# liyi14/mx-DeepIM

Hardware: NVIDIA H100
Metric: 480x640 4-iter pose refinements/sec (higher is better)
Workload: dtype fp16

## Files before the change

### mx-deepim_b200/csrc/conv_igemm.cuh

```cuda
#pragma once
#include <cuda.h>
#include <cuda_fp16.h>
#include "common.cuh"
#include "wgmma.cuh"

namespace dim {

struct ConvKParams {
  CUtensorMap a_map[4];
  CUtensorMap a_lo_map[4];
  CUtensorMap b_map;
  CUtensorMap b_lo_map;
  int KH, KW, stride, cchunks;
  int BW, BH, n_col_tiles;
  int Hq, Ho, Wo, Bn;
  int out_Hp, out_Wp, out_py, out_px, Cout;
  int kblocks;
  float slope;
  const float *bias;
  __nv_bfloat16 *out_hi, *out_lo;
  int in_off_r, in_off_c;
  int out_sy, out_sx, out_oy, out_ox, out_H, out_W, out_cs, out_coff;
  struct PixBuf { const __nv_bfloat16 *p; int Hp, Wp, py, px, cs, coff; } addend, mask;
  int mask_climit;
};

namespace ptx {
// ... 57 lines not shown
        : "memory");
}
__device__ __forceinline__ void tma_load_3d(void *dst, const CUtensorMap *map, uint64_t *bar, int c0, int c1, int c2) {
  if (elect_one())
    asm volatile(
        "cp.async.bulk.tensor.3d.shared::cluster.global.mbarrier::complete_tx::bytes [%0], [%1, {%3, %4, %5}], [%2];" ::
            "r"(smem_u32(dst)),
        "l"((uint64_t)map), "r"(smem_u32(bar)), "r"(c0), "r"(c1), "r"(c2)
        : "memory");
}

__device__ __forceinline__ void mbar_arrive(uint64_t *bar) {
  asm volatile("mbarrier.arrive.shared::cta.b64 _, [%0];" ::"r"(smem_u32(bar)) : "memory");
}

__device__ __forceinline__ void tma_load_4d(void *dst, const CUtensorMap *map, uint64_t *bar, int c0, int c1, int c2, int c3) {
  if (elect_one())
    asm volatile(
        "cp.async.bulk.tensor.4d.shared::cluster.global.mbarrier::complete_tx::bytes [%0], [%1, {%3, %4, %5, %6}], [%2];" ::
            "r"(smem_u32(dst)),
        "l"((uint64_t)map), "r"(smem_u32(bar)), "r"(c0), "r"(c1), "r"(c2), "r"(c3)
        : "memory");
}

__device__ __forceinline__ uint64_t gmma_desc(uint32_t saddr, uint32_t lbo_bytes, uint32_t sbo_bytes, uint32_t layout) {
  uint64_t d = 0;
  d |= (uint64_t)((saddr & 0x3FFFFu) >> 4);
  d |= (uint64_t)((lbo_bytes >> 4) & 0x3FFFu) << 16;
  d |= (uint64_t)((sbo_bytes >> 4) & 0x3FFFu) << 32;
  d |= (uint64_t)layout << 62;
// ... 11 lines not shown
  asm("cvt.rn.satfinite.f16x2.f32 %0, %1, %2;" : "=r"(r) : "f"(b), "f"(a));
  return r;
}
__device__ __forceinline__ uint32_t pack2_bf16(float a, float b) {
  uint32_t r;
  asm("cvt.rn.bf16x2.f32 %0, %1, %2;" : "=r"(r) : "f"(b), "f"(a));
  return r;
}

constexpr int kConv1Slack = 2048;


__device__ __forceinline__ int frag_row(int t) { return ((t >> 5) << 4) + ((t & 31) >> 2); }

template <bool SPLIT3, bool F16>
__device__ __forceinline__ void store_pair(float v0, float v1, float2 b, float slope, __nv_bfloat16 *out_hi, __nv_bfloat16 *out_lo,
                                           long long off) {
  v0 += b.x;
  v1 += b.y;
  v0 = v0 > 0.f ? v0 : v0 * slope;
  v1 = v1 > 0.f ? v1 : v1 * slope;
  if (F16) {
    *reinterpret_cast<uint32_t *>(out_hi + off) = pack2_f16(v0, v1);
  } else {
    const uint32_t h = pack2_bf16(v0, v1);
    *reinterpret_cast<uint32_t *>(out_hi + off) = h;
    if (SPLIT3)
      *reinterpret_cast<uint32_t *>(out_lo + off) = pack2_bf16(v0 - __uint_as_float(h << 16), v1 - __uint_as_float(h & 0xFFFF0000u));
  }
}

__device__ __forceinline__ void store_pair_generic(float v0, float v1, const ConvKParams &p, int n, bool valid, long long off,
                                                   long long add_off, long long mask_off) {
  if (!valid || n >= p.Cout) return;
  if (p.bias) {
    v0 += __ldg(p.bias + n);
    v1 += __ldg(p.bias + n + 1);
  }
  if (p.addend.p) {
    const __nv_bfloat162 a = *reinterpret_cast<const __nv_bfloat162 *>(p.addend.p + add_off);
    v0 += __low2float(a);
    v1 += __high2float(a);
  }
  if (p.mask.p) {
// ... 146 lines not shown
          const bool valid = (m < p.BW * p.BH) && (n_img < p.Bn) && (oh < p.Ho) && (ow < p.Wo);
          if (valid) {
            const long long off = (((long long)n_img * p.out_Hp + oh + p.out_py) * p.out_Wp + ow + p.out_px) * p.Cout + n0 + q2;
#pragma unroll
            for (int j = 0; j < BLOCK_N / 8; ++j)
              store_pair<SPLIT3, F16>(acc[4 * j + 2 * rr], acc[4 * j + 2 * rr + 1],
                                      make_float2(__ldg(p.bias + n0 + 8 * j + q2), __ldg(p.bias + n0 + 8 * j + q2 + 1)), p.slope, p.out_hi,
                                      p.out_lo, off + 8 * j);
          }
        }
      }
    }
  }
}

template <int STAGES, bool SPLIT3, bool F16>
__global__ void __launch_bounds__(384, 1) conv1_kernel(const __grid_constant__ ConvKParams p, const int rows_total,
                                                       const int rows_per_chunk, const int chunks_per_col,
                                                       const int strip_bytes ) {
  constexpr int NPREC = SPLIT3 ? 2 : 1;
  constexpr int B_BYTES = 64 * 32 * 2, RES_BYTES = 16 * B_BYTES * NPREC;
  extern __shared__ uint8_t smem_raw[];
  uint8_t *smem = reinterpret_cast<uint8_t *>((reinterpret_cast<uintptr_t>(smem_raw) + 1023) & ~(uintptr_t)1023);
  uint8_t *res = smem;
  uint8_t *ring = smem + RES_BYTES;
  const int stage_bytes = strip_bytes * NPREC;
  uint64_t *full_bar = reinterpret_cast<uint64_t *>(ring + STAGES * stage_bytes + kConv1Slack);
  uint64_t *empty_bar = full_bar + STAGES;
  uint64_t *res_bar = empty_bar + STAGES;

  const int wgi = threadIdx.x >> 7, warp = threadIdx.x >> 5;
  const int R = p.BW + 3;
  const uint32_t LBO = (uint32_t)R * 16u;
  const int ct = blockIdx.x / chunks_per_col, ck = blockIdx.x - ct * chunks_per_col;
  const int g_lo = ck * rows_per_chunk;
  const int g_hi = min(rows_total, g_lo + rows_per_chunk);
  const int n_rows = max(0, g_hi - g_lo);
  const int n_strips = n_rows > 0 ? n_rows + 3 : 0;
  const int ow0 = ct * p.BW;

  if (threadIdx.x == 0) {
    for (int s = 0; s < STAGES; ++s) {
      ptx::mbar_init(&full_bar[s], 1);
      ptx::mbar_init(&empty_bar[s], 2);
    }
    ptx::mbar_init(res_bar, 1);
    ptx::fence_barrier_init();
    ptx::prefetch_tmap(&p.b_map);
    ptx::prefetch_tmap(&p.a_map[0]);
  }
  __syncthreads();

  if (wgi == 0) {
    ptx::regs_producer();
    if (warp == 0 && n_rows > 0) {
      if (ptx::elect_one()) {
        ptx::mbar_expect_tx_raw(res_bar, (uint32_t)RES_BYTES);
        for (int kb = 0; kb < 16; ++kb) {
          ptx::tma_load_2d_raw(res + kb * B_BYTES, &p.b_map, res_bar, kb * 32, 0);
          if (SPLIT3) ptx::tma_load_2d_raw(res + (16 + kb) * B_BYTES, &p.b_lo_map, res_bar, kb * 32, 0);
        }
      }
      __syncwarp();
      const uint32_t tx = (uint32_t)(R * 64) * NPREC;
      for (int s = 0; s < n_strips; ++s) {
        const int slot = s % STAGES;
        ptx::mbar_wait(&empty_bar[slot], (((uint32_t)(s / STAGES)) & 1u) ^ 1u);
        uint8_t *st = ring + slot * stage_bytes;
        ptx::mbar_expect_tx(&full_bar[slot], tx);
        ptx::tma_load_4d(st, &p.a_map[0], &full_bar[slot], 0, ow0, 0, g_lo + s);
        if (SPLIT3) ptx::tma_load_4d(st + strip_bytes, &p.a_lo_map[0], &full_bar[slot], 0, ow0, 0, g_lo + s);
      }
    }
  } else if (n_rows > 0) {
    ptx::regs_consumer();
    const int set = wgi - 1, t = threadIdx.x & 127;
    const bool arriver = t == 0;
    const int r0 = frag_row(t), q2 = (t & 3) * 2;
    float2 bias[8];
#pragma unroll
    for (int j = 0; j < 8; ++j) bias[j] = make_float2(__ldg(p.bias + 8 * j + q2), __ldg(p.bias + 8 * j + q2 + 1));
    const uint32_t ring_a = ptx::smem_u32(ring);
    const uint64_t dring = ptx::gmma_desc(ring_a, LBO, 128, ptx::kNoSwizzle);
    const uint64_t dring3 = ptx::gmma_desc(ring_a, 2u * LBO, 128, ptx::kNoSwizzle) + 3u;
    const uint64_t lo_step = (uint64_t)((uint32_t)strip_bytes >> 4);
    const uint64_t slot_step = (uint64_t)((uint32_t)stage_bytes >> 4);
    const uint64_t kstep = (uint64_t)(2u * LBO >> 4);
    const uint64_t dres = ptx::gmma_desc(ptx::smem_u32(res), 16, 512, ptx::kSW64);
    const uint64_t dres_lo = dres + (uint64_t)((16 * B_BYTES) >> 4);
    const int n_cols_valid = min(p.BW, p.Wo - ow0);
    ptx::mbar_wait(res_bar, 0);
    if (set == 1 && arriver) ptx::mbar_arrive(&empty_bar[0]);
    for (int row = set; row < n_rows; row += 2) {
      float acc[2][32];
#pragma unroll
      for (int dh = 0; dh < 4; ++dh) {
        const int s = row + dh;
        ptx::mbar_wait(&full_bar[s % STAGES], ((uint32_t)(s / STAGES)) & 1u);
      }
      wg::fence_acc(acc[0]);
      wg::fence_acc(acc[1]);
      wg::fence();
#pragma unroll
      for (int h = 0; h < 2; ++h) {
#pragma unroll
        for (int dh = 0; dh < 4; ++dh) {
          const uint64_t so = (uint64_t)((row + dh) % STAGES) * slot_step + (uint64_t)(h * 64);
#pragma unroll
          for (int k = 0; k < 2; ++k) {
#pragma unroll
            for (int dw = 0; dw < 4; ++dw) {
              if ((dh == 3 || dw == 3) && k == 1) continue;
              const uint64_t da = (dw == 3 ? dring3 : dring + (uint64_t)dw + (uint64_t)k * kstep) + so;
              const uint64_t wo = (uint64_t)((dh * 4 + dw) * (B_BYTES >> 4) + 2 * k);
              wg::mma<64, F16, 0, 0>(acc[h], da, dres + wo, (dh | dw | k) ? 1u : 0u);
              if (SPLIT3) {
                wg::mma<64, false, 0, 0>(acc[h], da + lo_step, dres + wo, 1u);
                wg::mma<64, false, 0, 0>(acc[h], da, dres_lo + wo, 1u);
              }
            }
          }
        }
      }
      wg::commit();
      wg::wait<0>();
      wg::fence_acc(acc[0]);
      wg::fence_acc(acc[1]);
      if (arriver) {
        ptx::mbar_arrive(&empty_bar[row % STAGES]);
        ptx::mbar_arrive(&empty_bar[(row + 1) % STAGES]);
      }
      const int g = g_lo + row;
      const int n_img = g / p.Hq, oh = g - n_img * p.Hq;
      if (n_img < p.Bn && oh < p.Ho) {
        const long long row_off = (((long long)n_img * p.out_Hp + oh + p.out_py) * p.out_Wp + ow0 + p.out_px) * 64 + q2;
#pragma unroll
        for (int h = 0; h < 2; ++h)
#pragma unroll
          for (int rr = 0; rr < 2; ++rr) {
            const int m = h * 64 + r0 + rr * 8;
            if (m < n_cols_valid) {
#pragma unroll
              for (int j = 0; j < 8; ++j)
                store_pair<SPLIT3, F16>(acc[h][4 * j + 2 * rr], acc[h][4 * j + 2 * rr + 1], bias[j], p.slope, p.out_hi, p.out_lo,
                                        row_off + (long long)m * 64 + 8 * j);
            }
          }
      }
    }
  }
}

template <int STAGES, bool SPLIT3, bool F16, int NB>
__global__ void __launch_bounds__(384, 1) conv1_rgbd_kernel(const __grid_constant__ ConvKParams p, const int rows_total,
                                                            const int rows_per_chunk, const int chunks_per_col,
                                                            const int strip_bytes ) {
  constexpr int NPREC = SPLIT3 ? 2 : 1;
  constexpr int TAP_BYTES = NB * 128, RES_BYTES = 16 * TAP_BYTES * NPREC;
  extern __shared__ uint8_t smem_raw[];
  uint8_t *smem = reinterpret_cast<uint8_t *>((reinterpret_cast<uintptr_t>(smem_raw) + 1023) & ~(uintptr_t)1023);
  uint8_t *res = smem;
  uint8_t *ring = smem + RES_BYTES;
  const int stage_bytes = strip_bytes * NPREC;
  uint64_t *full_bar = reinterpret_cast<uint64_t *>(ring + STAGES * stage_bytes + kConv1Slack);
// ... 131 lines not shown
```

### mx-deepim_b200/csrc/net.cu

```cuda
#include <cuda_fp16.h>
#include <string.h>

#include <mutex>

#include "launch.cuh"
#include "net_state.cuh"

namespace dim {

static void build_geometry(NetState *ns, int H, int W) {
  int h = H, w = W;
  for (int i = 0; i < 10; ++i) {
    const LayerSpec &s = kLayers[i];
    LayerGeom &g = ns->g[i];
    g.Cin = s.Cin; g.Cout = s.Cout; g.k = s.k; g.stride = s.stride; g.pad = s.pad;
    g.Hin = h; g.Win = w;
    g.Ho = (h + 2 * s.pad - s.k) / s.stride + 1;
    g.Wo = (w + 2 * s.pad - s.k) / s.stride + 1;
    if (g.Ho < 1) g.Ho = 1;
    if (g.Wo < 1) g.Wo = 1;
    int Hp = h + 2 * s.pad, Wp = w + 2 * s.pad;
    if (s.stride == 2) { Hp += Hp & 1; Wp += Wp & 1; }
    g.py = g.px = s.pad;
    if (i == 0 && ns->input_depth) {
// ... 71 lines not shown
  for (int i = 0; i < 10; ++i) {
    const LayerGeom &g = ns->g[i];
    ConvKParams &kp = tm.kp[i];
    memset(&kp, 0, sizeof(kp));
    for (int lo = 0; lo < 2; ++lo) {
      __nv_bfloat16 *base = lo ? ns->act_lo[i] : ns->act_hi[i];
      CUtensorMap *maps = lo ? kp.a_lo_map : kp.a_map;
      const uint32_t box[3] = {(uint32_t)g.BLOCK_K, (uint32_t)g.BW, (uint32_t)g.BH};
      if (i == 0 && ns->input_depth) {
        const uint64_t dims[4] = {8, (uint64_t)g.cols, 8, (uint64_t)B * g.rows};
        const uint64_t str[3] = {16, (uint64_t)g.cols * 16, (uint64_t)g.cols * 128};
        const uint32_t box4[4] = {8, (uint32_t)(g.BW + 3), 8, 1};
        if (int rc = encode_map(&maps[0], base, 4, dims, str, box4, 0)) return rc;
        maps[1] = maps[2] = maps[3] = maps[0];
      } else if (i == 0) {
        const uint64_t dims[4] = {8, (uint64_t)g.cols, 4, (uint64_t)B * g.rows};
        const uint64_t str[3] = {16, (uint64_t)g.cols * 16, (uint64_t)g.cols * 64};
        const uint32_t box4[4] = {8, (uint32_t)(g.BW + 3), 4, 1};
        if (int rc = encode_map(&maps[0], base, 4, dims, str, box4, 0)) return rc;
        maps[1] = maps[2] = maps[3] = maps[0];
      } else if (g.stride_eff == 1) {
        const uint64_t dims[3] = {(uint64_t)g.Cbuf, (uint64_t)g.cols, (uint64_t)B * g.rows};
        const uint64_t str[2] = {(uint64_t)g.Cbuf * 2, (uint64_t)g.cols * g.Cbuf * 2};
        if (int rc = encode_map(&maps[0], base, 3, dims, str, box, g.BLOCK_K)) return rc;
        maps[1] = maps[2] = maps[3] = maps[0];
      } else {
        for (int ph = 0; ph < 2; ++ph)
          for (int pw = 0; pw < 2; ++pw) {
            const uint64_t dims[3] = {(uint64_t)g.Cbuf, (uint64_t)g.cols / 2, (uint64_t)B * g.rows / 2};
            const uint64_t str[2] = {(uint64_t)2 * g.Cbuf * 2, (uint64_t)2 * g.cols * g.Cbuf * 2};
            __nv_bfloat16 *vb = base + ((size_t)ph * g.cols + pw) * g.Cbuf;
            if (int rc = encode_map(&maps[(ph << 1) | pw], vb, 3, dims, str, box, g.BLOCK_K)) return rc;
          }
      }
    }
// ... 9 lines not shown
    kp.KH = g.KH; kp.KW = g.KW; kp.stride = g.stride_eff; kp.cchunks = g.Ceff / g.BLOCK_K;
    kp.BW = g.BW; kp.BH = g.BH; kp.n_col_tiles = g.n_col_tiles;
    kp.Hq = g.Hq; kp.Ho = g.Ho; kp.Wo = g.Wo; kp.Bn = B;
    if (i < 9) {
      const LayerGeom &nx = ns->g[i + 1];
      kp.out_Hp = nx.rows; kp.out_Wp = nx.cols; kp.out_py = nx.py; kp.out_px = nx.px;
    } else {
      kp.out_Hp = g.Ho; kp.out_Wp = g.Wo; kp.out_py = 0; kp.out_px = 0;
    }
    kp.Cout = g.Cout;
    kp.kblocks = g.kblocks;
    kp.slope = 0.1f;
    kp.bias = ns->bias[i];
    kp.out_hi = ns->act_hi[i + 1];
    kp.out_lo = ns->act_lo[i + 1];
  }
  return 0;
}

template <bool F16>
__device__ __forceinline__ void mma_bf16_16816(float *c, const uint32_t *a, uint32_t b0, uint32_t b1) {
  if (F16)
    asm volatile(
        "mma.sync.aligned.m16n8k16.row.col.f32.f16.f16.f32 {%0,%1,%2,%3}, {%4,%5,%6,%7}, {%8,%9}, {%0,%1,%2,%3};"
        : "+f"(c[0]), "+f"(c[1]), "+f"(c[2]), "+f"(c[3])
        : "r"(a[0]), "r"(a[1]), "r"(a[2]), "r"(a[3]), "r"(b0), "r"(b1));
  else
    asm volatile(
        "mma.sync.aligned.m16n8k16.row.col.f32.bf16.bf16.f32 {%0,%1,%2,%3}, {%4,%5,%6,%7}, {%8,%9}, {%0,%1,%2,%3};"
        : "+f"(c[0]), "+f"(c[1]), "+f"(c[2]), "+f"(c[3])
// ... 281 lines not shown
template <int BN, int ST, bool S3, bool F16>
static int launch_conv(const ConvKParams &kp, int total_tiles, int n_tiles, int cap, cudaStream_t st) {
  using S = ConvSmem2<BN, ST, S3>;
  static bool attr_set = false;
  if (!attr_set) {
    DIM_CHECK(cudaFuncSetAttribute(conv_igemm_persistent_kernel<BN, ST, S3, F16>, cudaFuncAttributeMaxDynamicSharedMemorySize,
                                   S::TOTAL));
    attr_set = true;
  }
  const int grid = total_tiles < cap ? total_tiles : cap;
  conv_igemm_persistent_kernel<BN, ST, S3, F16><<<grid, 384, S::TOTAL, st>>>(kp, total_tiles, n_tiles);
  DIM_LAUNCH_CHECK();
  return 0;
}

template <int ST, bool S3, bool F16>
static int launch_conv1(const ConvKParams &kp, int grid, int rows_total, int rpc, int chunks, int strip_bytes, cudaStream_t st) {
  const int smem_bytes = (S3 ? 2 : 1) * 16 * 4096 + ST * (S3 ? 2 : 1) * strip_bytes + kConv1Slack + 1024 + 256;
  DIM_REQUIRE(smem_bytes <= 227 * 1024, "conv1: image too wide for the rolling-strip ring");
  static int set = 0;
  if (set < smem_bytes) {
    DIM_CHECK(cudaFuncSetAttribute(conv1_kernel<ST, S3, F16>, cudaFuncAttributeMaxDynamicSharedMemorySize, smem_bytes));
    set = smem_bytes;
  }
  conv1_kernel<ST, S3, F16><<<grid, 384, smem_bytes, st>>>(kp, rows_total, rpc, chunks, strip_bytes);
  DIM_LAUNCH_CHECK();
  return 0;
}

template <int ST, bool S3, bool F16, int NB>
static int launch_conv1_rgbd(const ConvKParams &kp, int grid, int rows_total, int rpc, int chunks, int strip_bytes,
                             cudaStream_t st) {
  const int smem_bytes = 16 * NB * 128 * (S3 ? 2 : 1) + ST * (S3 ? 2 : 1) * strip_bytes + kConv1Slack + 1024 + 256;
  DIM_REQUIRE(smem_bytes <= 227 * 1024, "conv1 (RGB-D): image too wide for the rolling-strip ring");
  static int set = 0;
  if (set < smem_bytes) {
    DIM_CHECK(cudaFuncSetAttribute(conv1_rgbd_kernel<ST, S3, F16, NB>, cudaFuncAttributeMaxDynamicSharedMemorySize,
                                   smem_bytes));
    set = smem_bytes;
  }
// ... 62 lines not shown
    int rc;
    if (i == 0 && ns->input_depth) {
      const int nsplit = s3 ? 4 : 1;
      const int rows_total = B * g.Hq;
      int chunks = sms / (g.n_col_tiles * nsplit);
      if (chunks > cdiv(rows_total, 16)) chunks = cdiv(rows_total, 16);
      if (chunks < 1) chunks = 1;
      const int rpc = cdiv(rows_total, chunks);
      chunks = cdiv(rows_total, rpc);
      const int strip_bytes = cdiv((g.BW + 3) * 128, 128) * 128;
      const int grid = g.n_col_tiles * chunks * nsplit;
      rc = s3 ? launch_conv1_rgbd<5, true, false, 16>(kp, grid, rows_total, rpc, chunks, strip_bytes, st)
              : (f16 ? launch_conv1_rgbd<6, false, true, 64>(kp, grid, rows_total, rpc, chunks, strip_bytes, st)
                     : launch_conv1_rgbd<6, false, false, 64>(kp, grid, rows_total, rpc, chunks, strip_bytes, st));
    } else if (i == 0) {
      const int rows_total = B * g.Hq;
      int chunks = sms / g.n_col_tiles;
      if (chunks > cdiv(rows_total, 16)) chunks = cdiv(rows_total, 16);
      if (chunks < 1) chunks = 1;
      const int rpc = cdiv(rows_total, chunks);
      chunks = cdiv(rows_total, rpc);
      const int strip_bytes = cdiv((g.BW + 3) * 64, 128) * 128;
      const int grid = g.n_col_tiles * chunks;
      rc = s3 ? launch_conv1<5, true, false>(kp, grid, rows_total, rpc, chunks, strip_bytes, st)
              : (f16 ? launch_conv1<8, false, true>(kp, grid, rows_total, rpc, chunks, strip_bytes, st)
                     : launch_conv1<8, false, false>(kp, grid, rows_total, rpc, chunks, strip_bytes, st));
    } else if (g.BLOCK_N == 128) {
      rc = s3 ? launch_conv<128, 3, true, false>(kp, total_tiles, n_tiles, sms, st)
              : (f16 ? launch_conv<128, 6, false, true>(kp, total_tiles, n_tiles, sms, st)
                     : launch_conv<128, 6, false, false>(kp, total_tiles, n_tiles, sms, st));
    } else {
      rc = s3 ? launch_conv<256, 2, true, false>(kp, total_tiles, n_tiles, sms, st)
              : (f16 ? launch_conv<256, 4, false, true>(kp, total_tiles, n_tiles, sms, st)
                     : launch_conv<256, 4, false, false>(kp, total_tiles, n_tiles, sms, st));
    }
    if (rc) return rc;
    if (ns->layer_events && i < 9) DIM_CHECK(cudaEventRecord(ns->layer_events[i + 1], st));
  }
  if (ns->layer_events) DIM_CHECK(cudaEventRecord(ns->layer_events[10], st));
  if (after_conv) DIM_CHECK(cudaEventRecord(after_conv, st));
  if (s3)
// ... 63 lines not shown
```

### mx-deepim_b200/csrc/wgmma.cuh

```cuda
#pragma once
#include <stdint.h>

namespace dim {
namespace wg {

__device__ __forceinline__ void fence() { asm volatile("wgmma.fence.sync.aligned;" ::: "memory"); }
__device__ __forceinline__ void commit() { asm volatile("wgmma.commit_group.sync.aligned;" ::: "memory"); }
template <int N>
__device__ __forceinline__ void wait() { asm volatile("wgmma.wait_group.sync.aligned %0;" ::"n"(N) : "memory"); }

template <int R>
__device__ __forceinline__ void fence_acc(float (&d)[R]) {
#pragma unroll
  for (int i = 0; i < R; ++i) asm volatile("" : "+f"(d[i])::"memory");
}

template <int N, bool F16, int TA, int TB>
__device__ __forceinline__ void mma(float (&d)[N / 2], uint64_t da, uint64_t db, uint32_t scale_d);

template <>
__device__ __forceinline__ void mma<16, false, 0, 0>(float (&d)[8], uint64_t da, uint64_t db, uint32_t scale_d) {
  asm volatile(
      "{\n.reg .pred p;\nsetp.ne.b32 p, %10, 0;\n"
      "wgmma.mma_async.sync.aligned.m64n16k16.f32.bf16.bf16 {%0, %1, %2, %3, %4, %5, %6, %7}, %8, %9, p, 1, 1, 0, 0;\n}\n"
// ... 44 lines not shown
      "wgmma.mma_async.sync.aligned.m64n64k16.f32.f16.f16 {%0, %1, %2, %3, %4, %5, %6, %7, %8, %9, %10, %11, %12, %13, %14, %15, %16, %17, %18, %19, %20, %21, %22, %23, %24, %25, %26, %27, %28, %29, %30, %31}, %32, %33, p, 1, 1, 0, 0;\n}\n"
      : "+f"(d[0]), "+f"(d[1]), "+f"(d[2]), "+f"(d[3]), "+f"(d[4]), "+f"(d[5]), "+f"(d[6]), "+f"(d[7]), "+f"(d[8]), "+f"(d[9]), "+f"(d[10]), "+f"(d[11]), "+f"(d[12]), "+f"(d[13]), "+f"(d[14]), "+f"(d[15]), "+f"(d[16]), "+f"(d[17]), "+f"(d[18]), "+f"(d[19]), "+f"(d[20]), "+f"(d[21]), "+f"(d[22]), "+f"(d[23]), "+f"(d[24]), "+f"(d[25]), "+f"(d[26]), "+f"(d[27]), "+f"(d[28]), "+f"(d[29]), "+f"(d[30]), "+f"(d[31])
      : "l"(da), "l"(db), "r"(scale_d));
}

template <>
__device__ __forceinline__ void mma<64, false, 1, 1>(float (&d)[32], uint64_t da, uint64_t db, uint32_t scale_d) {
  asm volatile(
      "{\n.reg .pred p;\nsetp.ne.b32 p, %34, 0;\n"
      "wgmma.mma_async.sync.aligned.m64n64k16.f32.bf16.bf16 {%0, %1, %2, %3, %4, %5, %6, %7, %8, %9, %10, %11, %12, %13, %14, %15, %16, %17, %18, %19, %20, %21, %22, %23, %24, %25, %26, %27, %28, %29, %30, %31}, %32, %33, p, 1, 1, 1, 1;\n}\n"
      : "+f"(d[0]), "+f"(d[1]), "+f"(d[2]), "+f"(d[3]), "+f"(d[4]), "+f"(d[5]), "+f"(d[6]), "+f"(d[7]), "+f"(d[8]), "+f"(d[9]), "+f"(d[10]), "+f"(d[11]), "+f"(d[12]), "+f"(d[13]), "+f"(d[14]), "+f"(d[15]), "+f"(d[16]), "+f"(d[17]), "+f"(d[18]), "+f"(d[19]), "+f"(d[20]), "+f"(d[21]), "+f"(d[22]), "+f"(d[23]), "+f"(d[24]), "+f"(d[25]), "+f"(d[26]), "+f"(d[27]), "+f"(d[28]), "+f"(d[29]), "+f"(d[30]), "+f"(d[31])
      : "l"(da), "l"(db), "r"(scale_d));
}

template <>
__device__ __forceinline__ void mma<128, false, 0, 0>(float (&d)[64], uint64_t da, uint64_t db, uint32_t scale_d) {
  asm volatile(
      "{\n.reg .pred p;\nsetp.ne.b32 p, %66, 0;\n"
      "wgmma.mma_async.sync.aligned.m64n128k16.f32.bf16.bf16 {%0, %1, %2, %3, %4, %5, %6, %7, %8, %9, %10, %11, %12, %13, %14, %15, %16, %17, %18, %19, %20, %21, %22, %23, %24, %25, %26, %27, %28, %29, %30, %31, %32, %33, %34, %35, %36, %37, %38, %39, %40, %41, %42, %43, %44, %45, %46, %47, %48, %49, %50, %51, %52, %53, %54, %55, %56, %57, %58, %59, %60, %61, %62, %63}, %64, %65, p, 1, 1, 0, 0;\n}\n"
      : "+f"(d[0]), "+f"(d[1]), "+f"(d[2]), "+f"(d[3]), "+f"(d[4]), "+f"(d[5]), "+f"(d[6]), "+f"(d[7]), "+f"(d[8]), "+f"(d[9]), "+f"(d[10]), "+f"(d[11]), "+f"(d[12]), "+f"(d[13]), "+f"(d[14]), "+f"(d[15]), "+f"(d[16]), "+f"(d[17]), "+f"(d[18]), "+f"(d[19]), "+f"(d[20]), "+f"(d[21]), "+f"(d[22]), "+f"(d[23]), "+f"(d[24]), "+f"(d[25]), "+f"(d[26]), "+f"(d[27]), "+f"(d[28]), "+f"(d[29]), "+f"(d[30]), "+f"(d[31]), "+f"(d[32]), "+f"(d[33]), "+f"(d[34]), "+f"(d[35]), "+f"(d[36]), "+f"(d[37]), "+f"(d[38]), "+f"(d[39]), "+f"(d[40]), "+f"(d[41]), "+f"(d[42]), "+f"(d[43]), "+f"(d[44]), "+f"(d[45]), "+f"(d[46]), "+f"(d[47]), "+f"(d[48]), "+f"(d[49]), "+f"(d[50]), "+f"(d[51]), "+f"(d[52]), "+f"(d[53]), "+f"(d[54]), "+f"(d[55]), "+f"(d[56]), "+f"(d[57]), "+f"(d[58]), "+f"(d[59]), "+f"(d[60]), "+f"(d[61]), "+f"(d[62]), "+f"(d[63])
      : "l"(da), "l"(db), "r"(scale_d));
}

template <>
__device__ __forceinline__ void mma<128, true, 0, 0>(float (&d)[64], uint64_t da, uint64_t db, uint32_t scale_d) {
  asm volatile(
      "{\n.reg .pred p;\nsetp.ne.b32 p, %66, 0;\n"
      "wgmma.mma_async.sync.aligned.m64n128k16.f32.f16.f16 {%0, %1, %2, %3, %4, %5, %6, %7, %8, %9, %10, %11, %12, %13, %14, %15, %16, %17, %18, %19, %20, %21, %22, %23, %24, %25, %26, %27, %28, %29, %30, %31, %32, %33, %34, %35, %36, %37, %38, %39, %40, %41, %42, %43, %44, %45, %46, %47, %48, %49, %50, %51, %52, %53, %54, %55, %56, %57, %58, %59, %60, %61, %62, %63}, %64, %65, p, 1, 1, 0, 0;\n}\n"
      : "+f"(d[0]), "+f"(d[1]), "+f"(d[2]), "+f"(d[3]), "+f"(d[4]), "+f"(d[5]), "+f"(d[6]), "+f"(d[7]), "+f"(d[8]), "+f"(d[9]), "+f"(d[10]), "+f"(d[11]), "+f"(d[12]), "+f"(d[13]), "+f"(d[14]), "+f"(d[15]), "+f"(d[16]), "+f"(d[17]), "+f"(d[18]), "+f"(d[19]), "+f"(d[20]), "+f"(d[21]), "+f"(d[22]), "+f"(d[23]), "+f"(d[24]), "+f"(d[25]), "+f"(d[26]), "+f"(d[27]), "+f"(d[28]), "+f"(d[29]), "+f"(d[30]), "+f"(d[31]), "+f"(d[32]), "+f"(d[33]), "+f"(d[34]), "+f"(d[35]), "+f"(d[36]), "+f"(d[37]), "+f"(d[38]), "+f"(d[39]), "+f"(d[40]), "+f"(d[41]), "+f"(d[42]), "+f"(d[43]), "+f"(d[44]), "+f"(d[45]), "+f"(d[46]), "+f"(d[47]), "+f"(d[48]), "+f"(d[49]), "+f"(d[50]), "+f"(d[51]), "+f"(d[52]), "+f"(d[53]), "+f"(d[54]), "+f"(d[55]), "+f"(d[56]), "+f"(d[57]), "+f"(d[58]), "+f"(d[59]), "+f"(d[60]), "+f"(d[61]), "+f"(d[62]), "+f"(d[63])
      : "l"(da), "l"(db), "r"(scale_d));
// ... 41 lines not shown
```

Before: 2162.

## Transpose conv1 GEMM so weights are M and pixels N, with TMA-store epilogue

Result: faster. 2286, median of 6 (+5.7%).

```diff
diff --git a/mx-deepim_b200/csrc/conv_igemm.cuh b/mx-deepim_b200/csrc/conv_igemm.cuh
--- a/mx-deepim_b200/csrc/conv_igemm.cuh
+++ b/mx-deepim_b200/csrc/conv_igemm.cuh
@@ -11,6 +11,9 @@
   CUtensorMap a_lo_map[4];
   CUtensorMap b_map;
   CUtensorMap b_lo_map;
+  CUtensorMap out_map[2];
+  const __nv_bfloat16 *in_hi, *in_lo;
+  int in_cols;
   int KH, KW, stride, cchunks;
   int BW, BH, n_col_tiles;
   int Hq, Ho, Wo, Bn;
@@ -98,6 +101,28 @@
   asm volatile("mbarrier.arrive.shared::cta.b64 _, [%0];" ::"r"(smem_u32(bar)) : "memory");
 }
 
+__device__ __forceinline__ void bulk_load_raw(void *dst, const void *src, uint32_t bytes, uint64_t *bar) {
+  asm volatile("cp.async.bulk.shared::cluster.global.mbarrier::complete_tx::bytes [%0], [%1], %2, [%3];" ::"r"(smem_u32(dst)),
+               "l"(src), "r"(bytes), "r"(smem_u32(bar))
+               : "memory");
+}
+__device__ __forceinline__ void tma_store_4d(const CUtensorMap *map, const void *src, int c0, int c1, int c2, int c3) {
+  asm volatile("cp.async.bulk.tensor.4d.global.shared::cta.bulk_group [%0, {%2, %3, %4, %5}], [%1];" ::"l"((uint64_t)map),
+               "r"(smem_u32(src)), "r"(c0), "r"(c1), "r"(c2), "r"(c3)
+               : "memory");
+}
+__device__ __forceinline__ void bulk_commit() { asm volatile("cp.async.bulk.commit_group;" ::: "memory"); }
+__device__ __forceinline__ void bulk_wait_read0() { asm volatile("cp.async.bulk.wait_group.read 0;" ::: "memory"); }
+__device__ __forceinline__ void bulk_wait0() { asm volatile("cp.async.bulk.wait_group 0;" ::: "memory"); }
+__device__ __forceinline__ void named_bar_sync(int id, int threads) {
+  asm volatile("bar.sync %0, %1;" ::"r"(id), "r"(threads) : "memory");
+}
+__device__ __forceinline__ void stmatrix_x4_trans(uint32_t addr, const uint32_t (&r)[4]) {
+  asm volatile("stmatrix.sync.aligned.m8n8.x4.trans.shared.b16 [%0], {%1, %2, %3, %4};" ::"r"(addr), "r"(r[0]), "r"(r[1]),
+               "r"(r[2]), "r"(r[3])
+               : "memory");
+}
+
 __device__ __forceinline__ void tma_load_4d(void *dst, const CUtensorMap *map, uint64_t *bar, int c0, int c1, int c2, int c3) {
   if (elect_one())
     asm volatile(
@@ -139,20 +164,26 @@
 __device__ __forceinline__ int frag_row(int t) { return ((t >> 5) << 4) + ((t & 31) >> 2); }
 
 template <bool SPLIT3, bool F16>
-__device__ __forceinline__ void store_pair(float v0, float v1, float2 b, float slope, __nv_bfloat16 *out_hi, __nv_bfloat16 *out_lo,
-                                           long long off) {
-  v0 += b.x;
-  v1 += b.y;
+__device__ __forceinline__ void epi_pack(float v0, float v1, float b0, float b1, float slope, uint32_t &hi, uint32_t &lo) {
+  v0 += b0;
+  v1 += b1;
   v0 = v0 > 0.f ? v0 : v0 * slope;
   v1 = v1 > 0.f ? v1 : v1 * slope;
   if (F16) {
-    *reinterpret_cast<uint32_t *>(out_hi + off) = pack2_f16(v0, v1);
+    hi = pack2_f16(v0, v1);
   } else {
-    const uint32_t h = pack2_bf16(v0, v1);
-    *reinterpret_cast<uint32_t *>(out_hi + off) = h;
-    if (SPLIT3)
-      *reinterpret_cast<uint32_t *>(out_lo + off) = pack2_bf16(v0 - __uint_as_float(h << 16), v1 - __uint_as_float(h & 0xFFFF0000u));
-  }
+    hi = pack2_bf16(v0, v1);
+    if (SPLIT3) lo = pack2_bf16(v0 - __uint_as_float(hi << 16), v1 - __uint_as_float(hi & 0xFFFF0000u));
+  }
+}
+
+template <bool SPLIT3, bool F16>
+__device__ __forceinline__ void store_pair(float v0, float v1, float2 b, float slope, __nv_bfloat16 *out_hi, __nv_bfloat16 *out_lo,
+                                           long long off) {
+  uint32_t h, l = 0;
+  epi_pack<SPLIT3, F16>(v0, v1, b.x, b.y, slope, h, l);
+  *reinterpret_cast<uint32_t *>(out_hi + off) = h;
+  if (SPLIT3) *reinterpret_cast<uint32_t *>(out_lo + off) = l;
 }
 
 __device__ __forceinline__ void store_pair_generic(float v0, float v1, const ConvKParams &p, int n, bool valid, long long off,
@@ -329,30 +360,42 @@
   }
 }
 
-template <int STAGES, bool SPLIT3, bool F16>
+constexpr int kConv1StoreN = 80;
+
+template <int N, int STAGES, bool SPLIT3>
+struct Conv1Smem {
+  static constexpr int NPREC = SPLIT3 ? 2 : 1;
+  static constexpr int TAP_BYTES = 64 * 32 * 2;
+  static constexpr int RES_BYTES = 16 * TAP_BYTES * NPREC;
+  static constexpr int STG_BYTES = N * 128;
+  static constexpr int PLANE_BYTES = (N + 3) * 16;
+  static constexpr int STRIP_BYTES = (4 * PLANE_BYTES + 127) / 128 * 128;
+  static constexpr int STAGE_BYTES = STRIP_BYTES * NPREC;
+  static constexpr int TOTAL = RES_BYTES + 2 * STG_BYTES * NPREC + STAGES * STAGE_BYTES + 1024  + 256 ;
+  static_assert(N % kConv1StoreN == 0 && N % 16 == 0 && STG_BYTES % 1024 == 0, "conv1 tile width");
+  static_assert(TOTAL <= 227 * 1024, "conv1 shared memory");
+};
+
+template <int N, int STAGES, bool SPLIT3, bool F16>
 __global__ void __launch_bounds__(384, 1) conv1_kernel(const __grid_constant__ ConvKParams p, const int rows_total,
-                                                       const int rows_per_chunk, const int chunks_per_col,
-                                                       const int strip_bytes ) {
-  constexpr int NPREC = SPLIT3 ? 2 : 1;
-  constexpr int B_BYTES = 64 * 32 * 2, RES_BYTES = 16 * B_BYTES * NPREC;
+                                                       const int rows_per_chunk, const int chunks_per_col) {
+  using S = Conv1Smem<N, STAGES, SPLIT3>;
   extern __shared__ uint8_t smem_raw[];
   uint8_t *smem = reinterpret_cast<uint8_t *>((reinterpret_cast<uintptr_t>(smem_raw) + 1023) & ~(uintptr_t)1023);
   uint8_t *res = smem;
-  uint8_t *ring = smem + RES_BYTES;
-  const int stage_bytes = strip_bytes * NPREC;
-  uint64_t *full_bar = reinterpret_cast<uint64_t *>(ring + STAGES * stage_bytes + kConv1Slack);
+  uint8_t *stg = res + S::RES_BYTES;
+  uint8_t *ring = stg + 2 * S::NPREC * S::STG_BYTES;
+  uint64_t *full_bar = reinterpret_cast<uint64_t *>(ring + STAGES * S::STAGE_BYTES);
   uint64_t *empty_bar = full_bar + STAGES;
   uint64_t *res_bar = empty_bar + STAGES;
 
   const int wgi = threadIdx.x >> 7, warp = threadIdx.x >> 5;
-  const int R = p.BW + 3;
-  const uint32_t LBO = (uint32_t)R * 16u;
   const int ct = blockIdx.x / chunks_per_col, ck = blockIdx.x - ct * chunks_per_col;
   const int g_lo = ck * rows_per_chunk;
   const int g_hi = min(rows_total, g_lo + rows_per_chunk);
   const int n_rows = max(0, g_hi - g_lo);
   const int n_strips = n_rows > 0 ? n_rows + 3 : 0;
-  const int ow0 = ct * p.BW;
+  const int ow0 = ct * N;
 
   if (threadIdx.x == 0) {
     for (int s = 0; s < STAGES; ++s) {
@@ -362,7 +405,7 @@
     ptx::mbar_init(res_bar, 1);
     ptx::fence_barrier_init();
     ptx::prefetch_tmap(&p.b_map);
-    ptx::prefetch_tmap(&p.a_map[0]);
+    ptx::prefetch_tmap(&p.out_map[0]);
   }
   __syncthreads();
 
@@ -370,99 +413,117 @@
     ptx::regs_producer();
     if (warp == 0 && n_rows > 0) {
       if (ptx::elect_one()) {
-        ptx::mbar_expect_tx_raw(res_bar, (uint32_t)RES_BYTES);
+        ptx::mbar_expect_tx_raw(res_bar, (uint32_t)S::RES_BYTES);
         for (int kb = 0; kb < 16; ++kb) {
-          ptx::tma_load_2d_raw(res + kb * B_BYTES, &p.b_map, res_bar, kb * 32, 0);
-          if (SPLIT3) ptx::tma_load_2d_raw(res + (16 + kb) * B_BYTES, &p.b_lo_map, res_bar, kb * 32, 0);
+          ptx::tma_load_2d_raw(res + kb * S::TAP_BYTES, &p.b_map, res_bar, kb * 32, 0);
+          if (SPLIT3) ptx::tma_load_2d_raw(res + (16 + kb) * S::TAP_BYTES, &p.b_lo_map, res_bar, kb * 32, 0);
         }
       }
       __syncwarp();
-      const uint32_t tx = (uint32_t)(R * 64) * NPREC;
+      const size_t plane = (size_t)p.in_cols * 16;
+      const uint8_t *src_hi = reinterpret_cast<const uint8_t *>(p.in_hi) + (size_t)ow0 * 16;
+      const uint8_t *src_lo = reinterpret_cast<const uint8_t *>(p.in_lo) + (size_t)ow0 * 16;
       for (int s = 0; s < n_strips; ++s) {
         const int slot = s % STAGES;
         ptx::mbar_wait(&empty_bar[slot], (((uint32_t)(s / STAGES)) & 1u) ^ 1u);
-        uint8_t *st = ring + slot * stage_bytes;
-        ptx::mbar_expect_tx(&full_bar[slot], tx);
-        ptx::tma_load_4d(st, &p.a_map[0], &full_bar[slot], 0, ow0, 0, g_lo + s);
-        if (SPLIT3) ptx::tma_load_4d(st + strip_bytes, &p.a_lo_map[0], &full_bar[slot], 0, ow0, 0, g_lo + s);
+        uint8_t *st = ring + slot * S::STAGE_BYTES;
+        if (g_lo + s >= rows_total) {
+          if (ptx::elect_one()) ptx::mbar_arrive(&full_bar[slot]);
+        } else if (ptx::elect_one()) {
+          ptx::mbar_expect_tx_raw(&full_bar[slot], (uint32_t)(4 * S::PLANE_BYTES * S::NPREC));
+          const size_t row = (size_t)(g_lo + s) * 4 * plane;
+#pragma unroll
+          for (int c = 0; c < 4; ++c) {
+            ptx::bulk_load_raw(st + c * S::PLANE_BYTES, src_hi + row + c * plane, S::PLANE_BYTES, &full_bar[slot]);
+            if (SPLIT3)
+              ptx::bulk_load_raw(st + S::STRIP_BYTES + c * S::PLANE_BYTES, src_lo + row + c * plane, S::PLANE_BYTES, &full_bar[slot]);
+          }
+        }
+        __syncwarp();
       }
     }
   } else if (n_rows > 0) {
     ptx::regs_consumer();
-    const int set = wgi - 1, t = threadIdx.x & 127;
-    const bool arriver = t == 0;
-    const int r0 = frag_row(t), q2 = (t & 3) * 2;
-    float2 bias[8];
-#pragma unroll
-    for (int j = 0; j < 8; ++j) bias[j] = make_float2(__ldg(p.bias + 8 * j + q2), __ldg(p.bias + 8 * j + q2 + 1));
+    const int set = wgi - 1, t = threadIdx.x & 127, lane = t & 31;
+    const bool leader = t == 0;
+    const int co = frag_row(t);
+    const float b0 = __ldg(p.bias + co), b1 = __ldg(p.bias + co + 8);
     const uint32_t ring_a = ptx::smem_u32(ring);
-    const uint64_t dring = ptx::gmma_desc(ring_a, LBO, 128, ptx::kNoSwizzle);
-    const uint64_t dring3 = ptx::gmma_desc(ring_a, 2u * LBO, 128, ptx::kNoSwizzle) + 3u;
-    const uint64_t lo_step = (uint64_t)((uint32_t)strip_bytes >> 4);
-    const uint64_t slot_step = (uint64_t)((uint32_t)stage_bytes >> 4);
-    const uint64_t kstep = (uint64_t)(2u * LBO >> 4);
+    const uint64_t dring = ptx::gmma_desc(ring_a, S::PLANE_BYTES, 128, ptx::kNoSwizzle);
+    const uint64_t dring3 = ptx::gmma_desc(ring_a, 2u * S::PLANE_BYTES, 128, ptx::kNoSwizzle) + 3u;
+    const uint64_t lo_step = (uint64_t)(S::STRIP_BYTES >> 4);
+    const uint64_t slot_step = (uint64_t)(S::STAGE_BYTES >> 4);
+    const uint64_t kstep = (uint64_t)(2 * S::PLANE_BYTES >> 4);
     const uint64_t dres = ptx::gmma_desc(ptx::smem_u32(res), 16, 512, ptx::kSW64);
-    const uint64_t dres_lo = dres + (uint64_t)((16 * B_BYTES) >> 4);
-    const int n_cols_valid = min(p.BW, p.Wo - ow0);
+    const uint64_t dres_lo = dres + (uint64_t)((16 * S::TAP_BYTES) >> 4);
+    uint8_t *my_stg = stg + set * S::NPREC * S::STG_BYTES;
+    const int st_px = ((lane >> 4) << 3) + (lane & 7), st_chunk = 2 * (t >> 5) + ((lane >> 3) & 1);
+    const uint32_t st_addr = ptx::smem_u32(my_stg) + (uint32_t)(st_px * 128 + ((st_chunk ^ (lane & 7)) << 4));
     ptx::mbar_wait(res_bar, 0);
-    if (set == 1 && arriver) ptx::mbar_arrive(&empty_bar[0]);
+    if (set == 1 && leader) ptx::mbar_arrive(&empty_bar[0]);
     for (int row = set; row < n_rows; row += 2) {
-      float acc[2][32];
+      float acc[N / 2];
 #pragma unroll
       for (int dh = 0; dh < 4; ++dh) {
         const int s = row + dh;
         ptx::mbar_wait(&full_bar[s % STAGES], ((uint32_t)(s / STAGES)) & 1u);
       }
-      wg::fence_acc(acc[0]);
-      wg::fence_acc(acc[1]);
+      wg::fence_acc(acc);
       wg::fence();
 #pragma unroll
-      for (int h = 0; h < 2; ++h) {
-#pragma unroll
-        for (int dh = 0; dh < 4; ++dh) {
-          const uint64_t so = (uint64_t)((row + dh) % STAGES) * slot_step + (uint64_t)(h * 64);
-#pragma unroll
-          for (int k = 0; k < 2; ++k) {
-#pragma unroll
-            for (int dw = 0; dw < 4; ++dw) {
-              if ((dh == 3 || dw == 3) && k == 1) continue;
-              const uint64_t da = (dw == 3 ? dring3 : dring + (uint64_t)dw + (uint64_t)k * kstep) + so;
-              const uint64_t wo = (uint64_t)((dh * 4 + dw) * (B_BYTES >> 4) + 2 * k);
-              wg::mma<64, F16, 0, 0>(acc[h], da, dres + wo, (dh | dw | k) ? 1u : 0u);
-              if (SPLIT3) {
-                wg::mma<64, false, 0, 0>(acc[h], da + lo_step, dres + wo, 1u);
-                wg::mma<64, false, 0, 0>(acc[h], da, dres_lo + wo, 1u);
-              }
+      for (int dh = 0; dh < 4; ++dh) {
+        const uint64_t so = (uint64_t)((row + dh) % STAGES) * slot_step;
+#pragma unroll
+        for (int k = 0; k < 2; ++k) {
+#pragma unroll
+          for (int dw = 0; dw < 4; ++dw) {
+            if ((dh == 3 || dw == 3) && k == 1) continue;
+            const uint64_t db = (dw == 3 ? dring3 : dring + (uint64_t)dw + (uint64_t)k * kstep) + so;
+            const uint64_t wo = (uint64_t)((dh * 4 + dw) * (S::TAP_BYTES >> 4) + 2 * k);
+            wg::mma<N, F16, 0, 0>(acc, dres + wo, db, (dh | dw | k) ? 1u : 0u);
+            if (SPLIT3) {
+              wg::mma<N, false, 0, 0>(acc, dres + wo, db + lo_step, 1u);
+              wg::mma<N, false, 0, 0>(acc, dres_lo + wo, db, 1u);
             }
           }
         }
       }
       wg::commit();
       wg::wait<0>();
-      wg::fence_acc(acc[0]);
-      wg::fence_acc(acc[1]);
-      if (arriver) {
+      wg::fence_acc(acc);
+      if (leader) {
         ptx::mbar_arrive(&empty_bar[row % STAGES]);
         ptx::mbar_arrive(&empty_bar[(row + 1) % STAGES]);
       }
       const int g = g_lo + row;
       const int n_img = g / p.Hq, oh = g - n_img * p.Hq;
       if (n_img < p.Bn && oh < p.Ho) {
-        const long long row_off = (((long long)n_img * p.out_Hp + oh + p.out_py) * p.out_Wp + ow0 + p.out_px) * 64 + q2;
-#pragma unroll
-        for (int h = 0; h < 2; ++h)
-#pragma unroll
-          for (int rr = 0; rr < 2; ++rr) {
-            const int m = h * 64 + r0 + rr * 8;
-            if (m < n_cols_valid) {
-#pragma unroll
-              for (int j = 0; j < 8; ++j)
-                store_pair<SPLIT3, F16>(acc[h][4 * j + 2 * rr], acc[h][4 * j + 2 * rr + 1], bias[j], p.slope, p.out_hi, p.out_lo,
-                                        row_off + (long long)m * 64 + 8 * j);
-            }
-          }
-      }
-    }
+        if (leader) ptx::bulk_wait_read0();
+        ptx::named_bar_sync(1 + set, 128);
+#pragma unroll
+        for (int i = 0; i < N / 16; ++i) {
+          uint32_t h[4], l[4] = {0, 0, 0, 0};
+          epi_pack<SPLIT3, F16>(acc[8 * i + 0], acc[8 * i + 1], b0, b0, p.slope, h[0], l[0]);
+          epi_pack<SPLIT3, F16>(acc[8 * i + 2], acc[8 * i + 3], b1, b1, p.slope, h[1], l[1]);
+          epi_pack<SPLIT3, F16>(acc[8 * i + 4], acc[8 * i + 5], b0, b0, p.slope, h[2], l[2]);
+          epi_pack<SPLIT3, F16>(acc[8 * i + 6], acc[8 * i + 7], b1, b1, p.slope, h[3], l[3]);
+          ptx::stmatrix_x4_trans(st_addr + (uint32_t)(i * 16 * 128), h);
+          if (SPLIT3) ptx::stmatrix_x4_trans(st_addr + (uint32_t)(S::STG_BYTES + i * 16 * 128), l);
+        }
+        ptx::fence_proxy_async();
+        ptx::named_bar_sync(1 + set, 128);
+        if (leader) {
+#pragma unroll
+          for (int q = 0; q < N / kConv1StoreN; ++q) {
+            ptx::tma_store_4d(&p.out_map[0], my_stg + q * kConv1StoreN * 128, 0, ow0 + q * kConv1StoreN, oh, n_img);
+            if (SPLIT3)
+              ptx::tma_store_4d(&p.out_map[1], my_stg + S::STG_BYTES + q * kConv1StoreN * 128, 0, ow0 + q * kConv1StoreN, oh, n_img);
+          }
+          ptx::bulk_commit();
+        }
+      }
+    }
+    if (leader) ptx::bulk_wait0();
   }
 }
 
diff --git a/mx-deepim_b200/csrc/net.cu b/mx-deepim_b200/csrc/net.cu
--- a/mx-deepim_b200/csrc/net.cu
+++ b/mx-deepim_b200/csrc/net.cu
@@ -109,11 +109,6 @@
         if (int rc = encode_map(&maps[0], base, 4, dims, str, box4, 0)) return rc;
         maps[1] = maps[2] = maps[3] = maps[0];
       } else if (i == 0) {
-        const uint64_t dims[4] = {8, (uint64_t)g.cols, 4, (uint64_t)B * g.rows};
-        const uint64_t str[3] = {16, (uint64_t)g.cols * 16, (uint64_t)g.cols * 64};
-        const uint32_t box4[4] = {8, (uint32_t)(g.BW + 3), 4, 1};
-        if (int rc = encode_map(&maps[0], base, 4, dims, str, box4, 0)) return rc;
-        maps[1] = maps[2] = maps[3] = maps[0];
       } else if (g.stride_eff == 1) {
         const uint64_t dims[3] = {(uint64_t)g.Cbuf, (uint64_t)g.cols, (uint64_t)B * g.rows};
         const uint64_t str[2] = {(uint64_t)g.Cbuf * 2, (uint64_t)g.cols * g.Cbuf * 2};
@@ -153,6 +148,18 @@
     kp.bias = ns->bias[i];
     kp.out_hi = ns->act_hi[i + 1];
     kp.out_lo = ns->act_lo[i + 1];
+    if (i == 0 && !ns->input_depth) {
+      const LayerGeom &nx = ns->g[1];
+      kp.in_hi = ns->act_hi[0];
+      kp.in_lo = ns->act_lo[0];
+      kp.in_cols = g.cols;
+      const uint64_t dims[4] = {64, (uint64_t)g.Wo, (uint64_t)g.Ho, (uint64_t)B};
+      const uint64_t str[3] = {128, (uint64_t)nx.cols * 128, (uint64_t)nx.rows * nx.cols * 128};
+      const uint32_t box[4] = {64, (uint32_t)kConv1StoreN, 1, 1};
+      const size_t interior = ((size_t)nx.py * nx.cols + nx.px) * 64;
+      for (int lo = 0; lo < 2; ++lo)
+        if (int rc = encode_map(&kp.out_map[lo], (lo ? ns->act_lo[1] : ns->act_hi[1]) + interior, 4, dims, str, box, 64)) return rc;
+    }
   }
   return 0;
 }
@@ -464,16 +471,15 @@
   return 0;
 }
 
-template <int ST, bool S3, bool F16>
-static int launch_conv1(const ConvKParams &kp, int grid, int rows_total, int rpc, int chunks, int strip_bytes, cudaStream_t st) {
-  const int smem_bytes = (S3 ? 2 : 1) * 16 * 4096 + ST * (S3 ? 2 : 1) * strip_bytes + kConv1Slack + 1024 + 256;
-  DIM_REQUIRE(smem_bytes <= 227 * 1024, "conv1: image too wide for the rolling-strip ring");
-  static int set = 0;
-  if (set < smem_bytes) {
-    DIM_CHECK(cudaFuncSetAttribute(conv1_kernel<ST, S3, F16>, cudaFuncAttributeMaxDynamicSharedMemorySize, smem_bytes));
-    set = smem_bytes;
-  }
-  conv1_kernel<ST, S3, F16><<<grid, 384, smem_bytes, st>>>(kp, rows_total, rpc, chunks, strip_bytes);
+template <int N, int ST, bool S3, bool F16>
+static int launch_conv1(const ConvKParams &kp, int grid, int rows_total, int rpc, int chunks, cudaStream_t st) {
+  using S = Conv1Smem<N, ST, S3>;
+  static bool set = false;
+  if (!set) {
+    DIM_CHECK(cudaFuncSetAttribute(conv1_kernel<N, ST, S3, F16>, cudaFuncAttributeMaxDynamicSharedMemorySize, S::TOTAL));
+    set = true;
+  }
+  conv1_kernel<N, ST, S3, F16><<<grid, 384, S::TOTAL, st>>>(kp, rows_total, rpc, chunks);
   DIM_LAUNCH_CHECK();
   return 0;
 }
@@ -566,17 +572,19 @@
               : (f16 ? launch_conv1_rgbd<6, false, true, 64>(kp, grid, rows_total, rpc, chunks, strip_bytes, st)
                      : launch_conv1_rgbd<6, false, false, 64>(kp, grid, rows_total, rpc, chunks, strip_bytes, st));
     } else if (i == 0) {
+      DIM_REQUIRE(g.Wo == 320 && g.cols >= g.Wo + 3 && g.Hq == g.rows && g.Hq == g.Ho + 3,
+                  "conv1_kernel is built for a 480x640 input (320 output columns)");
+      const int n_col = g.Wo / (s3 ? 80 : 160);
       const int rows_total = B * g.Hq;
-      int chunks = sms / g.n_col_tiles;
+      int chunks = sms / n_col;
       if (chunks > cdiv(rows_total, 16)) chunks = cdiv(rows_total, 16);
       if (chunks < 1) chunks = 1;
       const int rpc = cdiv(rows_total, chunks);
       chunks = cdiv(rows_total, rpc);
-      const int strip_bytes = cdiv((g.BW + 3) * 64, 128) * 128;
-      const int grid = g.n_col_tiles * chunks;
-      rc = s3 ? launch_conv1<5, true, false>(kp, grid, rows_total, rpc, chunks, strip_bytes, st)
-              : (f16 ? launch_conv1<8, false, true>(kp, grid, rows_total, rpc, chunks, strip_bytes, st)
-                     : launch_conv1<8, false, false>(kp, grid, rows_total, rpc, chunks, strip_bytes, st));
+      const int grid = n_col * chunks;
+      rc = s3 ? launch_conv1<80, 5, true, false>(kp, grid, rows_total, rpc, chunks, st)
+              : (f16 ? launch_conv1<160, 8, false, true>(kp, grid, rows_total, rpc, chunks, st)
+                     : launch_conv1<160, 8, false, false>(kp, grid, rows_total, rpc, chunks, st));
     } else if (g.BLOCK_N == 128) {
       rc = s3 ? launch_conv<128, 3, true, false>(kp, total_tiles, n_tiles, sms, st)
               : (f16 ? launch_conv<128, 6, false, true>(kp, total_tiles, n_tiles, sms, st)
diff --git a/mx-deepim_b200/csrc/wgmma.cuh b/mx-deepim_b200/csrc/wgmma.cuh
--- a/mx-deepim_b200/csrc/wgmma.cuh
+++ b/mx-deepim_b200/csrc/wgmma.cuh
@@ -82,6 +82,33 @@
 }
 
 template <>
+__device__ __forceinline__ void mma<80, false, 0, 0>(float (&d)[40], uint64_t da, uint64_t db, uint32_t scale_d) {
+  asm volatile(
+      "{\n.reg .pred p;\nsetp.ne.b32 p, %42, 0;\n"
+      "wgmma.mma_async.sync.aligned.m64n80k16.f32.bf16.bf16 {%0, %1, %2, %3, %4, %5, %6, %7, %8, %9, %10, %11, %12, %13, %14, %15, %16, %17, %18, %19, %20, %21, %22, %23, %24, %25, %26, %27, %28, %29, %30, %31, %32, %33, %34, %35, %36, %37, %38, %39}, %40, %41, p, 1, 1, 0, 0;\n}\n"
+      : "+f"(d[0]), "+f"(d[1]), "+f"(d[2]), "+f"(d[3]), "+f"(d[4]), "+f"(d[5]), "+f"(d[6]), "+f"(d[7]), "+f"(d[8]), "+f"(d[9]), "+f"(d[10]), "+f"(d[11]), "+f"(d[12]), "+f"(d[13]), "+f"(d[14]), "+f"(d[15]), "+f"(d[16]), "+f"(d[17]), "+f"(d[18]), "+f"(d[19]), "+f"(d[20]), "+f"(d[21]), "+f"(d[22]), "+f"(d[23]), "+f"(d[24]), "+f"(d[25]), "+f"(d[26]), "+f"(d[27]), "+f"(d[28]), "+f"(d[29]), "+f"(d[30]), "+f"(d[31]), "+f"(d[32]), "+f"(d[33]), "+f"(d[34]), "+f"(d[35]), "+f"(d[36]), "+f"(d[37]), "+f"(d[38]), "+f"(d[39])
+      : "l"(da), "l"(db), "r"(scale_d));
+}
+
+template <>
+__device__ __forceinline__ void mma<160, false, 0, 0>(float (&d)[80], uint64_t da, uint64_t db, uint32_t scale_d) {
+  asm volatile(
+      "{\n.reg .pred p;\nsetp.ne.b32 p, %82, 0;\n"
+      "wgmma.mma_async.sync.aligned.m64n160k16.f32.bf16.bf16 {%0, %1, %2, %3, %4, %5, %6, %7, %8, %9, %10, %11, %12, %13, %14, %15, %16, %17, %18, %19, %20, %21, %22, %23, %24, %25, %26, %27, %28, %29, %30, %31, %32, %33, %34, %35, %36, %37, %38, %39, %40, %41, %42, %43, %44, %45, %46, %47, %48, %49, %50, %51, %52, %53, %54, %55, %56, %57, %58, %59, %60, %61, %62, %63, %64, %65, %66, %67, %68, %69, %70, %71, %72, %73, %74, %75, %76, %77, %78, %79}, %80, %81, p, 1, 1, 0, 0;\n}\n"
+      : "+f"(d[0]), "+f"(d[1]), "+f"(d[2]), "+f"(d[3]), "+f"(d[4]), "+f"(d[5]), "+f"(d[6]), "+f"(d[7]), "+f"(d[8]), "+f"(d[9]), "+f"(d[10]), "+f"(d[11]), "+f"(d[12]), "+f"(d[13]), "+f"(d[14]), "+f"(d[15]), "+f"(d[16]), "+f"(d[17]), "+f"(d[18]), "+f"(d[19]), "+f"(d[20]), "+f"(d[21]), "+f"(d[22]), "+f"(d[23]), "+f"(d[24]), "+f"(d[25]), "+f"(d[26]), "+f"(d[27]), "+f"(d[28]), "+f"(d[29]), "+f"(d[30]), "+f"(d[31]), "+f"(d[32]), "+f"(d[33]), "+f"(d[34]), "+f"(d[35]), "+f"(d[36]), "+f"(d[37]), "+f"(d[38]), "+f"(d[39]), "+f"(d[40]), "+f"(d[41]), "+f"(d[42]), "+f"(d[43]), "+f"(d[44]), "+f"(d[45]), "+f"(d[46]), "+f"(d[47]), "+f"(d[48]), "+f"(d[49]), "+f"(d[50]), "+f"(d[51]), "+f"(d[52]), "+f"(d[53]), "+f"(d[54]), "+f"(d[55]), "+f"(d[56]), "+f"(d[57]), "+f"(d[58]), "+f"(d[59]), "+f"(d[60]), "+f"(d[61]), "+f"(d[62]), "+f"(d[63]), "+f"(d[64]), "+f"(d[65]), "+f"(d[66]), "+f"(d[67]), "+f"(d[68]), "+f"(d[69]), "+f"(d[70]), "+f"(d[71]), "+f"(d[72]), "+f"(d[73]), "+f"(d[74]), "+f"(d[75]), "+f"(d[76]), "+f"(d[77]), "+f"(d[78]), "+f"(d[79])
+      : "l"(da), "l"(db), "r"(scale_d));
+}
+
+template <>
+__device__ __forceinline__ void mma<160, true, 0, 0>(float (&d)[80], uint64_t da, uint64_t db, uint32_t scale_d) {
+  asm volatile(
+      "{\n.reg .pred p;\nsetp.ne.b32 p, %82, 0;\n"
+      "wgmma.mma_async.sync.aligned.m64n160k16.f32.f16.f16 {%0, %1, %2, %3, %4, %5, %6, %7, %8, %9, %10, %11, %12, %13, %14, %15, %16, %17, %18, %19, %20, %21, %22, %23, %24, %25, %26, %27, %28, %29, %30, %31, %32, %33, %34, %35, %36, %37, %38, %39, %40, %41, %42, %43, %44, %45, %46, %47, %48, %49, %50, %51, %52, %53, %54, %55, %56, %57, %58, %59, %60, %61, %62, %63, %64, %65, %66, %67, %68, %69, %70, %71, %72, %73, %74, %75, %76, %77, %78, %79}, %80, %81, p, 1, 1, 0, 0;\n}\n"
+      : "+f"(d[0]), "+f"(d[1]), "+f"(d[2]), "+f"(d[3]), "+f"(d[4]), "+f"(d[5]), "+f"(d[6]), "+f"(d[7]), "+f"(d[8]), "+f"(d[9]), "+f"(d[10]), "+f"(d[11]), "+f"(d[12]), "+f"(d[13]), "+f"(d[14]), "+f"(d[15]), "+f"(d[16]), "+f"(d[17]), "+f"(d[18]), "+f"(d[19]), "+f"(d[20]), "+f"(d[21]), "+f"(d[22]), "+f"(d[23]), "+f"(d[24]), "+f"(d[25]), "+f"(d[26]), "+f"(d[27]), "+f"(d[28]), "+f"(d[29]), "+f"(d[30]), "+f"(d[31]), "+f"(d[32]), "+f"(d[33]), "+f"(d[34]), "+f"(d[35]), "+f"(d[36]), "+f"(d[37]), "+f"(d[38]), "+f"(d[39]), "+f"(d[40]), "+f"(d[41]), "+f"(d[42]), "+f"(d[43]), "+f"(d[44]), "+f"(d[45]), "+f"(d[46]), "+f"(d[47]), "+f"(d[48]), "+f"(d[49]), "+f"(d[50]), "+f"(d[51]), "+f"(d[52]), "+f"(d[53]), "+f"(d[54]), "+f"(d[55]), "+f"(d[56]), "+f"(d[57]), "+f"(d[58]), "+f"(d[59]), "+f"(d[60]), "+f"(d[61]), "+f"(d[62]), "+f"(d[63]), "+f"(d[64]), "+f"(d[65]), "+f"(d[66]), "+f"(d[67]), "+f"(d[68]), "+f"(d[69]), "+f"(d[70]), "+f"(d[71]), "+f"(d[72]), "+f"(d[73]), "+f"(d[74]), "+f"(d[75]), "+f"(d[76]), "+f"(d[77]), "+f"(d[78]), "+f"(d[79])
+      : "l"(da), "l"(db), "r"(scale_d));
+}
+
+template <>
 __device__ __forceinline__ void mma<128, false, 0, 0>(float (&d)[64], uint64_t da, uint64_t db, uint32_t scale_d) {
   asm volatile(
       "{\n.reg .pred p;\nsetp.ne.b32 p, %66, 0;\n"
```
